# Dave-he/unet-watermark

Hardware: AMD Instinct MI355X
Metric: train_images_per_sec (higher is better)
Workload: dtype f32 storage and accumulation; the convolution products of the encoder and decoder layers (3x3, 7x7 stem, stride-2 and 1x1 layers: forward, data gradients, and the weight gradients of the stride-1 3x3 layers and the stem) as fp16x3 splits - every fp32 operand = two fp16 halves (22 mantissa bits), a*b; 1 GPU; Unet-resnet34 512x512 bs16/GPU train step: fwd + Dice + bwd + Adam (BASELINE.json configs[1]); global_batch=16, parallelism=dp1, grad_allreduce=none

## Files before the change

unet-watermark_amd/csrc/wgrad_f16x3.hip:

```cpp
#include "uwm_kernels.h"

namespace uwm {

typedef float f4 __attribute__((ext_vector_type(4)));
typedef _Float16 h8 __attribute__((ext_vector_type(8)));
typedef _Float16 h4 __attribute__((ext_vector_type(4)));
typedef __fp16 fp16x4 __attribute__((__vector_size__(4 * sizeof(__fp16))));
typedef __attribute__((address_space(3))) fp16x4 lds_fp16x4;

#ifndef UWM_WG16_ABL
#define UWM_WG16_ABL 0
#endif
#ifndef UWM_WG16_XCD
#define UWM_WG16_XCD 1
#endif
template <int WX> struct WG16 {
  static constexpr int kWR = 128 / WX, kWX = WX, kWPW = WX + 2, kWPH = kWR + 2;
  static constexpr int kWXB = kWPH * kWPW * 136;
  static constexpr int kWStage = 32768 + ((kWXB + 255) & ~255);
  static constexpr int kWXRounds = (kWPH * kWPW * 8 + 511) / 512;
};
constexpr int kWDyB = 128 * 256;
constexpr int kWXS = 136;
constexpr int kWLT = 512;
constexpr int kWDyRounds = 128 * 16 / kWLT;

__device__ __forceinline__ int off_dy(int row, int ch) { return 256 * row + 16 * (ch ^ (((row & 3) << 2) | ((row >> 2) & 3))); }
__device__ __forceinline__ float clamp_hw(float v) { return __builtin_amdgcn_fmed3f(v, -65504.f, 65504.f); }
__device__ __forceinline__ h8 tr_pair(const char* base, int o0, int o1) {
  const fp16x4 lo = __builtin_amdgcn_ds_read_tr16_b64_v4f16((lds_fp16x4*)(uintptr_t)(base + o0));
  const fp16x4 hi = __builtin_amdgcn_ds_read_tr16_b64_v4f16((lds_fp16x4*)(uintptr_t)(base + o1));
  typedef __fp16 fp16x8 __attribute__((__vector_size__(8 * sizeof(__fp16))));
  const fp16x8 v = __builtin_shufflevector(lo, hi, 0, 1, 2, 3, 4, 5, 6, 7);
  return __builtin_bit_cast(h8, v);
}

template <int WX, int NP = 3>
__global__ __launch_bounds__(768, 1) void wgrad_f16x3_kernel(const WgradArgs a, int stages_per_split, int nstages) {
  constexpr int kWR = WG16<WX>::kWR, kWX = WX, kWPW = WG16<WX>::kWPW, kWPH = WG16<WX>::kWPH, kWStage = WG16<WX>::kWStage, kWXRounds = WG16<WX>::kWXRounds;
  constexpr int kKS = 4, kRK = 32 / WX;
  extern __shared__ __attribute__((aligned(256))) char wsm[];
  const int tid = threadIdx.x, lane = tid & 63, wave = __builtin_amdgcn_readfirstlane(tid >> 6);
  const bool is_mma = wave < 4;
  const int ltid = tid - 256;

  const int tilesA = (a.wrows + 63) / 64, tilesB = a.Ctot / 32;
  const int pairs = tilesA * tilesB;
#if UWM_WG16_XCD
  const unsigned nblk = gridDim.x, bid = blockIdx.x;
  const unsigned q8 = nblk >> 3, r8 = nblk & 7, xcd = bid & 7;
  const int lin = (int)((xcd < r8 ? xcd * (q8 + 1) : r8 * (q8 + 1) + (xcd - r8) * q8) + (bid >> 3));
#else
  const int lin = blockIdx.x;
#endif
  const int split = lin / pairs, pr = lin - split * pairs;
  const int ta = pr / tilesB, tb = pr - ta * tilesB;
  const int a0 = ta * 64, b0 = tb * 32;
  const int st0 = split * stages_per_split, st1 = min(nstages, st0 + stages_per_split);
  const int tilesX = a.Wo / kWX, tilesY = a.Ho / kWR;

  float xs = 1.f;
  if (a.xmax) {
    float mx = a.xmax[lane & 31];
#pragma unroll
    for (int d = 16; d >= 1; d >>= 1) mx = fmaxf(mx, __shfl_xor(mx, d));
    if (mx > 0.f && mx < 3.0e38f) { int e; (void)frexpf(mx, &e); xs = ldexpf(1.f, 14 - e); }
  }

  f4 acc[2][9];
#pragma unroll
  for (int cf = 0; cf < 2; ++cf)
#pragma unroll
    for (int t = 0; t < 9; ++t) acc[cf][t] = (f4){0.f, 0.f, 0.f, 0.f};

  if (!is_mma) {
    const bool first = b0 < a.C0;
    const Src& s = first ? a.s0 : a.s1;
    const int cl = first ? b0 : b0 - a.C0;
    const int dcu = ltid & 15;
    const bool dok = a0 + dcu * 4 < a.Cout;
    const int xcu = ltid & 7;
    f4 xsc = {1.f, 1.f, 1.f, 1.f}, xsh = {0.f, 0.f, 0.f, 0.f};
    const bool xhas = s.scale != nullptr;
    if (xhas) { xsc = *(const f4*)(s.scale + cl + xcu * 4); xsh = *(const f4*)(s.shift + cl + xcu * 4); }
    const int xrelu = s.relu;
    struct Stage { f4 dv[kWDyRounds]; f4 xv[kWXRounds]; unsigned xok; };
    int dgo[kWDyRounds], dlo[kWDyRounds], xpy[kWXRounds], xlo[kWXRounds];
#pragma unroll
    for (int rd = 0; rd < kWDyRounds; ++rd) {
      const int px = (rd * kWLT + ltid) >> 4;
      dgo[rd] = ((px / kWX) * a.Wo + (px % kWX)) * a.Cout;
      dlo[rd] = off_dy(px, dcu >> 1) + (dcu & 1) * 8;
    }
#pragma unroll
    for (int rd = 0; rd < kWXRounds; ++rd) {
      const int pp = (rd * kWLT + ltid) >> 3;
      const bool act = pp < kWPH * kWPW;
      const int py = act ? pp / kWPW : 0, px = act ? pp - py * kWPW : 0;
      xpy[rd] = act ? ((py << 8) | px) : -1;
      xlo[rd] = pp * kWXS + xcu * 8;
    }
    const float* const dyp = a.dy + a0 + dcu * 4;
    const float* const xp = s.ptr + cl + xcu * 4;
    auto stage_load = [&](int st, Stage& sg) {
      int q = st;
      const int tx = q % tilesX; q /= tilesX;
      const int ty = q % tilesY; const int n = q / tilesY;
      const int y0 = ty * kWR, x0 = tx * kWX;
      const float* const dbase = dyp + (((size_t)n * a.Ho + y0) * a.Wo + x0) * a.Cout;
#pragma unroll
      for (int rd = 0; rd < kWDyRounds; ++rd) sg.dv[rd] = dok ? *(const f4*)(dbase + dgo[rd]) : (f4){0.f, 0.f, 0.f, 0.f};
      sg.xok = 0;
      const int nb = n * s.H;
#pragma unroll
      for (int rd = 0; rd < kWXRounds; ++rd) {
        const int hl = y0 - 1 + (xpy[rd] >> 8), wl = x0 - 1 + (xpy[rd] & 255);
        const bool ok = xpy[rd] >= 0 && hl >= 0 && hl < a.Hl && wl >= 0 && wl < a.Wl;
        const int hc = min(max(hl, 0), a.Hl - 1), wc = min(max(wl, 0), a.Wl - 1);
        sg.xv[rd] = *(const f4*)(xp + (size_t)(((nb + (hc >> s.up)) * s.W + (wc >> s.up))) * s.C);
        sg.xok |= (ok ? 1u : 0u) << rd;
      }
    };
    auto split_store = [&](char* dst_hi, char* dst_lo, f4 v, bool clamp) {
      h4 hi, lo;
#pragma unroll
      for (int e = 0; e < 4; ++e) {
        const float x = clamp ? clamp_hw(v[e]) : v[e];
        const _Float16 h = (_Float16)x;
        hi[e] = h; lo[e] = (_Float16)(x - (float)h);
      }
      *(h4*)dst_hi = hi; *(h4*)dst_lo = lo;
    };
    auto stage_store = [&](int buf, const Stage& sg) {
      char* const dyb = wsm + buf * kWStage;
      char* const xb = dyb + kWDyB;
#pragma unroll
      for (int rd = 0; rd < kWDyRounds; ++rd) split_store(dyb + dlo[rd], dyb + (dlo[rd] ^ 128), sg.dv[rd] * xs, false);
#pragma unroll
      for (int rd = 0; rd < kWXRounds; ++rd) {
        if (xpy[rd] >= 0) {
          f4 v = sg.xv[rd];
          if (xhas) {
            v = v * xsc + xsh;
            if (xrelu) { v.x = fmaxf(v.x, 0.f); v.y = fmaxf(v.y, 0.f); v.z = fmaxf(v.z, 0.f); v.w = fmaxf(v.w, 0.f); }
          }
          if (!((sg.xok >> rd) & 1u)) v = (f4){0.f, 0.f, 0.f, 0.f};
          split_store(xb + xlo[rd], xb + xlo[rd] + 64, v, true);
        }
      }
    };
    Stage sA, sB;
    const int ns = st1 - st0;
    if (ns > 0) {
      stage_load(st0, sA);
      stage_load(ns > 1 ? st0 + 1 : st0, sB);
      stage_store(0, sA);
    }
    __syncthreads();
    constexpr bool skip = (UWM_WG16_ABL & 4) != 0;
    for (int i = 0; i < ns; i += 2) {
      {
        if (i + 1 < ns && !(skip && i > 0)) stage_store(1, sB);
        if (!skip) stage_load(st0 + (i + 2 < ns ? i + 2 : ns - 1), sA);
        __syncthreads();
      }
      if (i + 1 < ns) {
        if (i + 2 < ns && !skip) stage_store(0, sA);
        if (!skip) stage_load(st0 + (i + 3 < ns ? i + 3 : ns - 1), sB);
        __syncthreads();
      }
    }
  } else {
    const int cp = wave & 1, bf = wave >> 1;
    const int kg = lane >> 4, q = (lane & 15) >> 2, p = lane & 3;
    int dyo[2][2];
#pragma unroll
    for (int cf = 0; cf < 2; ++cf)
#pragma unroll
      for (int rdx = 0; rdx < 2; ++rdx)
        dyo[cf][rdx] = off_dy(8 * kg + 4 * rdx + q, 2 * (2 * cp + cf) + (p >> 1)) + 8 * (p & 1);
    const int xo = (((8 * kg) / kWX) * kWPW + (8 * kg) % kWX + q) * kWXS + (2 * bf + (p >> 1)) * 16 + 8 * (p & 1);
    const int ns = st1 - st0;
    __syncthreads();
    for (int i = 0; i < ns; ++i) {
      const char* const dyb = wsm + (i & 1) * kWStage;
      const char* const xb = dyb + kWDyB;
#pragma unroll
      for (int kr = 0; kr < kKS; ++kr) {
        h8 ah[2], al[2];
#pragma unroll
        for (int cf = 0; cf < 2; ++cf) {
          ah[cf] = tr_pair(dyb + kr * 32 * 256, dyo[cf][0], dyo[cf][1]);
          al[cf] = tr_pair(dyb + kr * 32 * 256, dyo[cf][0] ^ 128, dyo[cf][1] ^ 128);
        }
        h8 xh[3], xl[3];
        auto x_read = [&](int t) {
          const int r = t / 3, sx = t % 3;
          const char* xp = xb + ((kr * kRK + r) * kWPW + sx) * kWXS + xo;
          xh[t % 3] = (UWM_WG16_ABL & 2) ? ah[0] : tr_pair(xp, 0, 4 * kWXS);
          xl[t % 3] = (UWM_WG16_ABL & 2) ? al[1] : tr_pair(xp, 64, 4 * kWXS + 64);
        };
        x_read(0);
#pragma unroll
        for (int it = 0; it < 10; ++it) {
          if (it + 1 < 9) x_read(it + 1);
          if (UWM_WG16_ABL & 1) { if (it < 9) { acc[0][it][0] += (float)xh[it % 3][0] + (float)xl[it % 3][1]; acc[1][it][1] += (float)ah[1][2] + (float)al[0][3]; } continue; }
          const int pt = it - 1, ps = (it + 2) % 3, cs = it % 3;
          if (it < 9) acc[0][it] = __builtin_amdgcn_mfma_f32_16x16x32_f16(ah[0], xh[cs], acc[0][it], 0, 0, 0);
          if (NP >= 2 && it >= 1) acc[0][pt] = __builtin_amdgcn_mfma_f32_16x16x32_f16(ah[0], xl[ps], acc[0][pt], 0, 0, 0);
          if (it < 9) acc[1][it] = __builtin_amdgcn_mfma_f32_16x16x32_f16(ah[1], xh[cs], acc[1][it], 0, 0, 0);
          if (NP >= 2 && it >= 1) acc[1][pt] = __builtin_amdgcn_mfma_f32_16x16x32_f16(ah[1], xl[ps], acc[1][pt], 0, 0, 0);
          if (NP >= 3 && it >= 1) acc[0][pt] = __builtin_amdgcn_mfma_f32_16x16x32_f16(al[0], xh[ps], acc[0][pt], 0, 0, 0);
          if (NP >= 3 && it >= 1) acc[1][pt] = __builtin_amdgcn_mfma_f32_16x16x32_f16(al[1], xh[ps], acc[1][pt], 0, 0, 0);
          __builtin_amdgcn_sched_barrier(0);
        }
      }
      __syncthreads();
    }
    const float ixs = 1.f / xs;
    float* const dst = a.nsplit > 1 ? a.part + (size_t)split * a.wrows * a.Kpad : a.dw;
    const int ci = b0 + 16 * bf + (lane & 15);
#pragma unroll
    for (int cf = 0; cf < 2; ++cf)
#pragma unroll
      for (int t = 0; t < 9; ++t)
#pragma unroll
        for (int e = 0; e < 4; ++e) {
          const int row = a0 + 16 * (2 * cp + cf) + 4 * (lane >> 4) + e;
          if (row < a.wrows && ci < a.Ctot) {
            float* pd = dst + (size_t)row * a.Kpad + t * a.Ctot + ci;
            const float v = acc[cf][t][e] * ixs;
            if (UWM_WG16_ABL & 8) { if (v == 123.456f) *pd = v; }
            else if (a.nsplit > 1) *pd = v; else *pd += v;
          }
        }
  }
}

static int wgrad_f16x3_wx(const WgradArgs& a) {
  if ((a.Wo % 32) == 0 && (a.Ho % 4) == 0) return 32;
  if ((a.Wo % 16) == 0 && (a.Ho % 8) == 0) return 16;
  return 0;
}
bool wgrad_f16x3_applicable(const WgradArgs& a) {
  return a.xmax != nullptr && a.ntaps == 9 && a.kw == 3 && a.stride == 1 && a.pad == 1 && (a.Ctot & 31) == 0 && (a.C0 & 31) == 0 &&
         (a.Cout & 3) == 0 && a.wrows <= a.Cout && a.Kpad == 9 * a.Ctot && a.Hl == a.Ho && a.Wl == a.Wo &&
         wgrad_f16x3_wx(a) != 0 && (a.s0.C & 3) == 0 && (a.s1.C & 3) == 0 && a.Wo < 256 * 128 &&
         (size_t)a.N * a.s0.H * a.s0.W < (1ull << 31) && (size_t)a.N * a.s1.H * a.s1.W < (1ull << 31) && (size_t)8 * a.Wo * a.Cout < (1ull << 31);
}

template <int WX, int NP>
static hipError_t launch_wg16p(WgradArgs& a, hipStream_t st, int pairs, int sps, int nstages) {
  const size_t lds = (size_t)2 * WG16<WX>::kWStage;
  static DevOnce lds_attr;
  { hipError_t e = lds_attr.set_max_lds((const void*)wgrad_f16x3_kernel<WX, NP>, lds); if (e != hipSuccess) return e; }
  UWM_LAUNCH(43, a.flops, a.bytes, (wgrad_f16x3_kernel<WX, NP>), dim3((unsigned)(pairs * a.nsplit)), dim3(768), lds, st, a, sps, nstages);
  return hipGetLastError();
}
template <int WX>
static hipError_t launch_wg16(WgradArgs& a, hipStream_t st, int pairs, int sps, int nstages) {
  const int np = (a.nprod >= 1 && a.nprod <= 3) ? a.nprod : 3;
  return np == 3 ? launch_wg16p<WX, 3>(a, st, pairs, sps, nstages) : np == 2 ? launch_wg16p<WX, 2>(a, st, pairs, sps, nstages) : launch_wg16p<WX, 1>(a, st, pairs, sps, nstages);
}

hipError_t launch_wgrad_f16x3(const WgradArgs& a0, hipStream_t st) {
  WgradArgs a = a0;
  if (!wgrad_f16x3_applicable(a)) return hipErrorInvalidValue;
  const int wx = wgrad_f16x3_wx(a);
  const int pairs = ((a.wrows + 63) / 64) * (a.Ctot / 32);
  const int nstages = a.N * (a.Ho / (128 / wx)) * (a.Wo / wx);
  static const int cu_cap = dbg_int("UWM_WG16_CUS", 0);
  const int cus = cu_cap > 0 ? cu_cap : (a.cu_share > 0 ? device_cu_count() * a.cu_share / 4 : device_cu_count());
  int nsplit = (cus + pairs - 1) / pairs;
  if (nsplit > nstages / 4) nsplit = nstages / 4;
  if (nsplit < 1) nsplit = 1;
  const size_t image = (size_t)a.wrows * a.Kpad;
  if (nsplit > 1 && (!a.part || a.part_floats < 2 * image)) { a.part = wgrad_op_scratch(); a.part_floats = wgrad_wino_scratch_floats(); a.rq = nullptr; }
  if (nsplit > 1 && (!a.part || (size_t)nsplit * image > a.part_floats)) nsplit = a.part ? (int)(a.part_floats / image) : 1;
  if (nsplit < 1) nsplit = 1;
  const int sps = (nstages + nsplit - 1) / nsplit;
  nsplit = (nstages + sps - 1) / sps;
  a.nsplit = nsplit; a.msplit = sps;
  hipError_t e = wx == 32 ? launch_wg16<32>(a, st, pairs, sps, nstages) : launch_wg16<16>(a, st, pairs, sps, nstages);
  if (e != hipSuccess) return e;
  if (nsplit > 1) return launch_wgrad_reduce(a.part, nsplit, image / 4, a.dw, st, a.rq);
  return hipSuccess;
}

}
```

Measured before the change: 1195 images/s.

## Add narrow-output wgrad kernel tiling 32 output rows for small Cout layers

Adds a specialized fp16x3 weight-gradient kernel for layers with at most 32 output rows (wrows<=32) and 32-wide spatial tiles. It tiles input channels in 32 or 64 blocks with a 4x32 spatial tile, new LDS swizzles and split-tap MMA work across waves. The goal is to stop wasting half of each 64-row tile on small-Cout layers. It also changes the split count to round down (cus/pairs), which may lower grid fill.

New measurement: 1205 images/s, median of 6. About the same (+0.9%).

```diff
diff --git a/unet-watermark_amd/csrc/wgrad_f16x3.hip b/unet-watermark_amd/csrc/wgrad_f16x3.hip
--- a/unet-watermark_amd/csrc/wgrad_f16x3.hip
+++ b/unet-watermark_amd/csrc/wgrad_f16x3.hip
@@ -35,6 +35,26 @@
   return __builtin_bit_cast(h8, v);
 }
 
+__device__ __forceinline__ int wg16_lin() {
+#if UWM_WG16_XCD
+  const unsigned nblk = gridDim.x, bid = blockIdx.x;
+  const unsigned q8 = nblk >> 3, r8 = nblk & 7, xcd = bid & 7;
+  return (int)((xcd < r8 ? xcd * (q8 + 1) : r8 * (q8 + 1) + (xcd - r8) * q8) + (bid >> 3));
+#else
+  return blockIdx.x;
+#endif
+}
+__device__ __forceinline__ void split_store(char* dst_hi, char* dst_lo, f4 v, bool clamp) {
+  h4 hi, lo;
+#pragma unroll
+  for (int e = 0; e < 4; ++e) {
+    const float x = clamp ? clamp_hw(v[e]) : v[e];
+    const _Float16 h = (_Float16)x;
+    hi[e] = h; lo[e] = (_Float16)(x - (float)h);
+  }
+  *(h4*)dst_hi = hi; *(h4*)dst_lo = lo;
+}
+
 template <int WX, int NP = 3>
 __global__ __launch_bounds__(768, 1) void wgrad_f16x3_kernel(const WgradArgs a, int stages_per_split, int nstages) {
   constexpr int kWR = WG16<WX>::kWR, kWX = WX, kWPW = WG16<WX>::kWPW, kWPH = WG16<WX>::kWPH, kWStage = WG16<WX>::kWStage, kWXRounds = WG16<WX>::kWXRounds;
@@ -46,13 +66,7 @@
 
   const int tilesA = (a.wrows + 63) / 64, tilesB = a.Ctot / 32;
   const int pairs = tilesA * tilesB;
-#if UWM_WG16_XCD
-  const unsigned nblk = gridDim.x, bid = blockIdx.x;
-  const unsigned q8 = nblk >> 3, r8 = nblk & 7, xcd = bid & 7;
-  const int lin = (int)((xcd < r8 ? xcd * (q8 + 1) : r8 * (q8 + 1) + (xcd - r8) * q8) + (bid >> 3));
-#else
-  const int lin = blockIdx.x;
-#endif
+  const int lin = wg16_lin();
   const int split = lin / pairs, pr = lin - split * pairs;
   const int ta = pr / tilesB, tb = pr - ta * tilesB;
   const int a0 = ta * 64, b0 = tb * 32;
@@ -121,16 +135,6 @@
         sg.xok |= (ok ? 1u : 0u) << rd;
       }
     };
-    auto split_store = [&](char* dst_hi, char* dst_lo, f4 v, bool clamp) {
-      h4 hi, lo;
-#pragma unroll
-      for (int e = 0; e < 4; ++e) {
-        const float x = clamp ? clamp_hw(v[e]) : v[e];
-        const _Float16 h = (_Float16)x;
-        hi[e] = h; lo[e] = (_Float16)(x - (float)h);
-      }
-      *(h4*)dst_hi = hi; *(h4*)dst_lo = lo;
-    };
     auto stage_store = [&](int buf, const Stage& sg) {
       char* const dyb = wsm + buf * kWStage;
       char* const xb = dyb + kWDyB;
@@ -237,6 +241,214 @@
   }
 }
 
+template <int CI> struct WG32 {
+  static constexpr int kXRB = 4 * CI;
+  static constexpr int kXB = 6 * 34 * kXRB;
+  static constexpr int kDyB = 128 * 128;
+  static constexpr int kStage = kDyB + kXB;
+  static constexpr int kQPP = CI / 4;
+  static constexpr int kXRounds = (6 * 34 * kQPP + kWLT - 1) / kWLT;
+  static constexpr int kDyRounds = 128 * 8 / kWLT;
+};
+__device__ __forceinline__ int off_dy32(int row, int s) { return 128 * row + 32 * (s ^ (((row >> 1) & 1) | ((((row >> 3) ^ (row >> 2)) & 1) << 1))); }
+template <int CI> __device__ __forceinline__ int off_x32(int pp, int x, int s) {
+  const int g = CI == 64 ? ((x & 3) | (((x >> 3) & 1) << 2)) : (((x >> 1) & 1) | (((x >> 3) & 1) << 1));
+  return WG32<CI>::kXRB * pp + 32 * (s ^ g);
+}
+
+template <int CI, int NP, int T0, int NT>
+__device__ __forceinline__ void wg32_mma(const WgradArgs& a, const char* wsm, int ns, int split, int b0, int bf, int lane, float xs) {
+  constexpr int kStage = WG32<CI>::kStage, kDyB = WG32<CI>::kDyB, kXRB = WG32<CI>::kXRB, kKS = 4, kWPW = 34;
+  f4 acc[2][NT];
+#pragma unroll
+  for (int cf = 0; cf < 2; ++cf)
+#pragma unroll
+    for (int t = 0; t < NT; ++t) acc[cf][t] = (f4){0.f, 0.f, 0.f, 0.f};
+  const int kg = lane >> 4, q = (lane & 15) >> 2, p = lane & 3;
+  int dyo[2][2];
+#pragma unroll
+  for (int cf = 0; cf < 2; ++cf)
+#pragma unroll
+    for (int rdx = 0; rdx < 2; ++rdx) dyo[cf][rdx] = off_dy32(8 * kg + 4 * rdx + q, cf) + 8 * p;
+  int xo[3][2];
+#pragma unroll
+  for (int sx = 0; sx < 3; ++sx)
+#pragma unroll
+    for (int rdx = 0; rdx < 2; ++rdx) { const int x = sx + 8 * kg + 4 * rdx + q; xo[sx][rdx] = off_x32<CI>(x, x, bf) + 8 * p; }
+  __syncthreads();
+  for (int i = 0; i < ns; ++i) {
+    const char* const dyb = wsm + (i & 1) * kStage;
+    const char* const xb = dyb + kDyB;
+#pragma unroll
+    for (int kr = 0; kr < kKS; ++kr) {
+      h8 ah[2], al[2];
+#pragma unroll
+      for (int cf = 0; cf < 2; ++cf) {
+        ah[cf] = tr_pair(dyb + kr * 32 * 128, dyo[cf][0], dyo[cf][1]);
+        al[cf] = tr_pair(dyb + kr * 32 * 128, dyo[cf][0] ^ 64, dyo[cf][1] ^ 64);
+      }
+      h8 xh[3], xl[3];
+      auto x_read = [&](int j) {
+        const int r = (T0 + j) / 3, sx = (T0 + j) % 3;
+        const char* xp = xb + (kr + r) * kWPW * kXRB;
+        xh[j % 3] = (UWM_WG16_ABL & 2) ? ah[0] : tr_pair(xp, xo[sx][0], xo[sx][1]);
+        xl[j % 3] = (UWM_WG16_ABL & 2) ? al[1] : tr_pair(xp, xo[sx][0] ^ (kXRB / 2), xo[sx][1] ^ (kXRB / 2));
+      };
+      x_read(0);
+#pragma unroll
+      for (int it = 0; it < NT + 1; ++it) {
+        if (it + 1 < NT) x_read(it + 1);
+        if (UWM_WG16_ABL & 1) { if (it < NT) { acc[0][it][0] += (float)xh[it % 3][0] + (float)xl[it % 3][1]; acc[1][it][1] += (float)ah[1][2] + (float)al[0][3]; } continue; }
+        const int pt = it - 1, ps = (it + 2) % 3, cs = it % 3;
+        if (it < NT) acc[0][it] = __builtin_amdgcn_mfma_f32_16x16x32_f16(ah[0], xh[cs], acc[0][it], 0, 0, 0);
+        if (NP >= 2 && it >= 1) acc[0][pt] = __builtin_amdgcn_mfma_f32_16x16x32_f16(ah[0], xl[ps], acc[0][pt], 0, 0, 0);
+        if (it < NT) acc[1][it] = __builtin_amdgcn_mfma_f32_16x16x32_f16(ah[1], xh[cs], acc[1][it], 0, 0, 0);
+        if (NP >= 2 && it >= 1) acc[1][pt] = __builtin_amdgcn_mfma_f32_16x16x32_f16(ah[1], xl[ps], acc[1][pt], 0, 0, 0);
+        if (NP >= 3 && it >= 1) acc[0][pt] = __builtin_amdgcn_mfma_f32_16x16x32_f16(al[0], xh[ps], acc[0][pt], 0, 0, 0);
+        if (NP >= 3 && it >= 1) acc[1][pt] = __builtin_amdgcn_mfma_f32_16x16x32_f16(al[1], xh[ps], acc[1][pt], 0, 0, 0);
+        __builtin_amdgcn_sched_barrier(0);
+      }
+    }
+    __syncthreads();
+  }
+  const float ixs = 1.f / xs;
+  float* const dst = a.nsplit > 1 ? a.part + (size_t)split * a.wrows * a.Kpad : a.dw;
+  const int ci = b0 + 16 * bf + (lane & 15);
+#pragma unroll
+  for (int cf = 0; cf < 2; ++cf)
+#pragma unroll
+    for (int t = 0; t < NT; ++t)
+#pragma unroll
+      for (int e = 0; e < 4; ++e) {
+        const int row = 16 * cf + 4 * (lane >> 4) + e;
+        if (row < a.wrows && ci < a.Ctot) {
+          float* pd = dst + (size_t)row * a.Kpad + (T0 + t) * a.Ctot + ci;
+          const float v = acc[cf][t][e] * ixs;
+          if (UWM_WG16_ABL & 8) { if (v == 123.456f) *pd = v; }
+          else if (a.nsplit > 1) *pd = v; else *pd += v;
+        }
+      }
+}
+
+template <int CI, int NP = 3>
+__global__ __launch_bounds__(768, 1) void wgrad_f16x3_kernel_co32(const WgradArgs a, int stages_per_split, int nstages) {
+  constexpr int kWR = 4, kWX = 32, kWPW = 34, kWPH = 6, kStage = WG32<CI>::kStage, kDyB = WG32<CI>::kDyB, kXRB = WG32<CI>::kXRB;
+  constexpr int kQPP = WG32<CI>::kQPP, kXRounds = WG32<CI>::kXRounds, kDyRounds = WG32<CI>::kDyRounds;
+  extern __shared__ __attribute__((aligned(256))) char wsm[];
+  const int tid = threadIdx.x, lane = tid & 63, wave = __builtin_amdgcn_readfirstlane(tid >> 6);
+  const int ltid = tid - 256;
+
+  const int pairs = a.Ctot / CI;
+  const int lin = wg16_lin();
+  const int split = lin / pairs, tb = lin - split * pairs;
+  const int b0 = tb * CI;
+  const int st0 = split * stages_per_split, st1 = min(nstages, st0 + stages_per_split);
+  const int ns = st1 - st0;
+  const int tilesX = a.Wo / kWX, tilesY = a.Ho / kWR;
+
+  float xs = 1.f;
+  if (a.xmax) {
+    float mx = a.xmax[lane & 31];
+#pragma unroll
+    for (int d = 16; d >= 1; d >>= 1) mx = fmaxf(mx, __shfl_xor(mx, d));
+    if (mx > 0.f && mx < 3.0e38f) { int e; (void)frexpf(mx, &e); xs = ldexpf(1.f, 14 - e); }
+  }
+
+  if (wave >= 4) {
+    const bool first = b0 < a.C0;
+    const Src& s = first ? a.s0 : a.s1;
+    const int cl = first ? b0 : b0 - a.C0;
+    const int dcu = ltid & 7;
+    const bool dok = dcu * 4 < a.Cout;
+    const int xcu = ltid & (kQPP - 1);
+    f4 xsc = {1.f, 1.f, 1.f, 1.f}, xsh = {0.f, 0.f, 0.f, 0.f};
+    const bool xhas = s.scale != nullptr;
+    if (xhas) { xsc = *(const f4*)(s.scale + cl + xcu * 4); xsh = *(const f4*)(s.shift + cl + xcu * 4); }
+    const int xrelu = s.relu;
+    struct Stage { f4 dv[kDyRounds]; f4 xv[kXRounds]; unsigned xok; };
+    int dgo[kDyRounds], dlo[kDyRounds], xpy[kXRounds], xlo[kXRounds];
+#pragma unroll
+    for (int rd = 0; rd < kDyRounds; ++rd) {
+      const int px = (rd * kWLT + ltid) >> 3;
+      dgo[rd] = ((px / kWX) * a.Wo + (px % kWX)) * a.Cout;
+      dlo[rd] = off_dy32(px, dcu >> 2) + (dcu & 3) * 8;
+    }
+#pragma unroll
+    for (int rd = 0; rd < kXRounds; ++rd) {
+      const int pp = (rd * kWLT + ltid) / kQPP;
+      const bool act = pp < kWPH * kWPW;
+      const int py = act ? pp / kWPW : 0, px = act ? pp - py * kWPW : 0;
+      xpy[rd] = act ? ((py << 8) | px) : -1;
+      xlo[rd] = off_x32<CI>(pp, px, xcu >> 2) + (xcu & 3) * 8;
+    }
+    const float* const dyp = a.dy + dcu * 4;
+    const float* const xp = s.ptr + cl + xcu * 4;
+    auto stage_load = [&](int st, Stage& sg) {
+      int q = st;
+      const int tx = q % tilesX; q /= tilesX;
+      const int ty = q % tilesY; const int n = q / tilesY;
+      const int y0 = ty * kWR, x0 = tx * kWX;
+      const float* const dbase = dyp + (((size_t)n * a.Ho + y0) * a.Wo + x0) * a.Cout;
+#pragma unroll
+      for (int rd = 0; rd < kDyRounds; ++rd) sg.dv[rd] = dok ? *(const f4*)(dbase + dgo[rd]) : (f4){0.f, 0.f, 0.f, 0.f};
+      sg.xok = 0;
+      const int nb = n * s.H;
+#pragma unroll
+      for (int rd = 0; rd < kXRounds; ++rd) {
+        const int hl = y0 - 1 + (xpy[rd] >> 8), wl = x0 - 1 + (xpy[rd] & 255);
+        const bool ok = xpy[rd] >= 0 && hl >= 0 && hl < a.Hl && wl >= 0 && wl < a.Wl;
+        const int hc = min(max(hl, 0), a.Hl - 1), wc = min(max(wl, 0), a.Wl - 1);
+        sg.xv[rd] = *(const f4*)(xp + (size_t)(((nb + (hc >> s.up)) * s.W + (wc >> s.up))) * s.C);
+        sg.xok |= (ok ? 1u : 0u) << rd;
+      }
+    };
+    auto stage_store = [&](int buf, const Stage& sg) {
+      char* const dyb = wsm + buf * kStage;
+      char* const xb = dyb + kDyB;
+#pragma unroll
+      for (int rd = 0; rd < kDyRounds; ++rd) split_store(dyb + dlo[rd], dyb + (dlo[rd] ^ 64), sg.dv[rd] * xs, false);
+#pragma unroll
+      for (int rd = 0; rd < kXRounds; ++rd) {
+        if (xpy[rd] >= 0) {
+          f4 v = sg.xv[rd];
+          if (xhas) {
+            v = v * xsc + xsh;
+            if (xrelu) { v.x = fmaxf(v.x, 0.f); v.y = fmaxf(v.y, 0.f); v.z = fmaxf(v.z, 0.f); v.w = fmaxf(v.w, 0.f); }
+          }
+          if (!((sg.xok >> rd) & 1u)) v = (f4){0.f, 0.f, 0.f, 0.f};
+          split_store(xb + xlo[rd], xb + (xlo[rd] ^ (kXRB / 2)), v, true);
+        }
+      }
+    };
+    Stage sA, sB;
+    if (ns > 0) {
+      stage_load(st0, sA);
+      stage_load(ns > 1 ? st0 + 1 : st0, sB);
+      stage_store(0, sA);
+    }
+    __syncthreads();
+    constexpr bool skip = (UWM_WG16_ABL & 4) != 0;
+    for (int i = 0; i < ns; i += 2) {
+      {
+        if (i + 1 < ns && !(skip && i > 0)) stage_store(1, sB);
+        if (!skip) stage_load(st0 + (i + 2 < ns ? i + 2 : ns - 1), sA);
+        __syncthreads();
+      }
+      if (i + 1 < ns) {
+        if (i + 2 < ns && !skip) stage_store(0, sA);
+        if (!skip) stage_load(st0 + (i + 3 < ns ? i + 3 : ns - 1), sB);
+        __syncthreads();
+      }
+    }
+  } else if (CI == 64) {
+    wg32_mma<CI, NP, 0, 9>(a, wsm, ns, split, b0, wave, lane, xs);
+  } else if (wave < 2) {
+    wg32_mma<CI, NP, 0, 5>(a, wsm, ns, split, b0, wave & 1, lane, xs);
+  } else {
+    wg32_mma<CI, NP, 5, 4>(a, wsm, ns, split, b0, wave & 1, lane, xs);
+  }
+}
+
 static int wgrad_f16x3_wx(const WgradArgs& a) {
   if ((a.Wo % 32) == 0 && (a.Ho % 4) == 0) return 32;
   if ((a.Wo % 16) == 0 && (a.Ho % 8) == 0) return 16;
@@ -263,15 +475,31 @@
   return np == 3 ? launch_wg16p<WX, 3>(a, st, pairs, sps, nstages) : np == 2 ? launch_wg16p<WX, 2>(a, st, pairs, sps, nstages) : launch_wg16p<WX, 1>(a, st, pairs, sps, nstages);
 }
 
+template <int CI, int NP>
+static hipError_t launch_wg32p(WgradArgs& a, hipStream_t st, int pairs, int sps, int nstages) {
+  const size_t lds = (size_t)2 * WG32<CI>::kStage;
+  static DevOnce lds_attr;
+  { hipError_t e = lds_attr.set_max_lds((const void*)wgrad_f16x3_kernel_co32<CI, NP>, lds); if (e != hipSuccess) return e; }
+  UWM_LAUNCH(43, a.flops, a.bytes, (wgrad_f16x3_kernel_co32<CI, NP>), dim3((unsigned)(pairs * a.nsplit)), dim3(768), lds, st, a, sps, nstages);
+  return hipGetLastError();
+}
+template <int CI>
+static hipError_t launch_wg32(WgradArgs& a, hipStream_t st, int pairs, int sps, int nstages) {
+  const int np = (a.nprod >= 1 && a.nprod <= 3) ? a.nprod : 3;
+  return np == 3 ? launch_wg32p<CI, 3>(a, st, pairs, sps, nstages) : np == 2 ? launch_wg32p<CI, 2>(a, st, pairs, sps, nstages) : launch_wg32p<CI, 1>(a, st, pairs, sps, nstages);
+}
+
 hipError_t launch_wgrad_f16x3(const WgradArgs& a0, hipStream_t st) {
   WgradArgs a = a0;
   if (!wgrad_f16x3_applicable(a)) return hipErrorInvalidValue;
   const int wx = wgrad_f16x3_wx(a);
-  const int pairs = ((a.wrows + 63) / 64) * (a.Ctot / 32);
+  static const bool no_co32 = dbg_flag("UWM_WG16_NO_CO32");
+  const int tile = (no_co32 || a.wrows > 32 || wx != 32) ? 0 : ((a.Ctot % 64) == 0 && (a.C0 % 64) == 0) ? 1 : 2;
+  const int pairs = tile == 1 ? a.Ctot / 64 : tile == 2 ? a.Ctot / 32 : ((a.wrows + 63) / 64) * (a.Ctot / 32);
   const int nstages = a.N * (a.Ho / (128 / wx)) * (a.Wo / wx);
   static const int cu_cap = dbg_int("UWM_WG16_CUS", 0);
   const int cus = cu_cap > 0 ? cu_cap : (a.cu_share > 0 ? device_cu_count() * a.cu_share / 4 : device_cu_count());
-  int nsplit = (cus + pairs - 1) / pairs;
+  int nsplit = cus / pairs;
   if (nsplit > nstages / 4) nsplit = nstages / 4;
   if (nsplit < 1) nsplit = 1;
   const size_t image = (size_t)a.wrows * a.Kpad;
@@ -281,7 +509,8 @@
   const int sps = (nstages + nsplit - 1) / nsplit;
   nsplit = (nstages + sps - 1) / sps;
   a.nsplit = nsplit; a.msplit = sps;
-  hipError_t e = wx == 32 ? launch_wg16<32>(a, st, pairs, sps, nstages) : launch_wg16<16>(a, st, pairs, sps, nstages);
+  hipError_t e = tile == 1 ? launch_wg32<64>(a, st, pairs, sps, nstages) : tile == 2 ? launch_wg32<32>(a, st, pairs, sps, nstages) :
+                 wx == 32 ? launch_wg16<32>(a, st, pairs, sps, nstages) : launch_wg16<16>(a, st, pairs, sps, nstages);
   if (e != hipSuccess) return e;
   if (nsplit > 1) return launch_wgrad_reduce(a.part, nsplit, image / 4, a.dw, st, a.rq);
   return hipSuccess;
```
